# siboehm/ShallowSpeed

Hardware: AMD Instinct MI355X
Metric: samples/sec (whole node), 4-layer MLP MNIST-shape, DP×PP at 1/2/4/8 GPUs (higher is better)
Workload: dtype bf16; 1 GPU; model=mlp4_mnist_784x256x256x256x10, global_batch=16384, parallelism=dp1, schedule=naive, loss=xent, mubatches=1, hipgraph=False, fp8_fwd=False, deterministic=False

## Files before the change

csrc/bindings.cpp:

```cpp

#include <torch/extension.h>

#include <ATen/cuda/CUDAContext.h>

#include <climits>
#include <optional>
#include <string>

#include "launchers.h"

namespace {

hipStream_t cur_stream() {
    return (hipStream_t)at::cuda::getCurrentCUDAStream().stream();
}

void check_bf16(const torch::Tensor& t, const char* name) {
    TORCH_CHECK(t.is_cuda(), name, " must be on GPU");
    TORCH_CHECK(t.scalar_type() == torch::kBFloat16, name, " must be bf16");
    TORCH_CHECK(t.is_contiguous(), name, " must be contiguous");
}

void check_f32(const torch::Tensor& t, const char* name) {
    TORCH_CHECK(t.is_cuda(), name, " must be on GPU");
// ... 168 lines not shown
                                          const torch::Tensor& bsc,
                                          const torch::Tensor& bias,
                                          bool relu) {
    TORCH_CHECK(a.scalar_type() == torch::kUInt8 &&
                b.scalar_type() == torch::kUInt8, "a/b must be u8 (e4m3)");
    TORCH_CHECK(a.is_contiguous() && b.is_contiguous() &&
                asc.is_contiguous() && bsc.is_contiguous(), "contiguous");
    const int M = a.size(0), K = a.size(1), N = b.size(0);
    TORCH_CHECK(b.size(1) == K, "K mismatch");
    const void* bias_p = opt_bf16(bias, "bias");
    std::vector<torch::Tensor> out;
    bool ok;
    if (quantized) {
        out = {torch::empty({M, N}, a.options()),
               torch::empty({N / 128, M, 4}, a.options())};
        ok = ss_gemm_nt_f8_q(a.data_ptr(), asc.data_ptr(), b.data_ptr(),
                             bsc.data_ptr(), bias_p, out[0].data_ptr(),
                             out[1].data_ptr(), M, N, K, relu, cur_stream());
    } else {
        out = {torch::empty({M, N}, a.options().dtype(torch::kBFloat16))};
        ok = ss_gemm_nt_f8(a.data_ptr(), asc.data_ptr(), b.data_ptr(),
                           bsc.data_ptr(), bias_p, out[0].data_ptr(), M, N, K,
                           relu, cur_stream());
    }
    TORCH_CHECK(ok, "shape outside the fp8 tier: ", M, "x", N, "x", K);
    return out;
}

torch::Tensor gemm_nt_f8(torch::Tensor a, torch::Tensor asc, torch::Tensor b,
                         torch::Tensor bsc, torch::Tensor bias, bool relu) {
    return gemm_nt_f8_any(false, a, asc, b, bsc, bias, relu)[0];
}

std::vector<torch::Tensor> gemm_nt_f8_q(torch::Tensor a, torch::Tensor asc,
                                         torch::Tensor b, torch::Tensor bsc,
                                         torch::Tensor bias, bool relu) {
    return gemm_nt_f8_any(true, a, asc, b, bsc, bias, relu);
}

void wgrad_tn_256(torch::Tensor dy, torch::Tensor x, torch::Tensor gw) {
    check_bf16(dy, "dy");
    check_bf16(x, "x");
    check_f32(gw, "gw");
    const int Kb = dy.size(0), Mo = dy.size(1), N = x.size(1);
    TORCH_CHECK(x.size(0) == Kb, "batch mismatch");
    TORCH_CHECK(gw.size(0) == Mo && gw.size(1) == N, "gw shape");
    TORCH_CHECK(ss_wgrad_tn_256(dy.data_ptr(), x.data_ptr(), gw.data_ptr(),
                                Mo, N, Kb, cur_stream()),
                "shape outside the 256-tile wgrad tier");
}

void wgrad_tn(torch::Tensor dy, torch::Tensor x, torch::Tensor gw,
              torch::Tensor gb, torch::Tensor mask, int64_t split_k,
              int64_t stages) {
    check_bf16(dy, "dy");
    check_bf16(x, "x");
    check_f32(gw, "gw");
    const int Kb = dy.size(0), Mo = dy.size(1), N = x.size(1);
    TORCH_CHECK(x.size(0) == Kb, "batch mismatch");
    TORCH_CHECK(gw.size(0) == Mo && gw.size(1) == N, "gw shape");
    const void* mask_p = opt_bf16(mask, "mask");
    TORCH_CHECK(!mask_p || mask.sizes() == dy.sizes(), "mask must match dy");
    void* gb_p = opt_f32(gb, "gb");
    TORCH_CHECK(!gb_p || gb.numel() == Mo, "gb size");
    TORCH_CHECK(stages >= 0 && stages <= 2, "stages must be 0, 1 or 2");
    ss_wgrad_tn(dy.data_ptr(), x.data_ptr(), mask_p, gw.data_ptr(), gb_p, Mo,
                N, Kb, (int)split_k, (int)stages, cur_stream());
}

void wgrad_tn_multi(torch::Tensor chunk_table, int64_t nchunks,
                    bool has_mask, torch::Tensor gw, torch::Tensor gb,
                    int64_t Mo, int64_t N, int64_t kb_chunk,
                    int64_t split_k) {
    check_table(chunk_table, 3, "chunk_table must be CUDA int64 [nchunks,3]");
    TORCH_CHECK(chunk_table.size(0) == nchunks,
                "chunk_table must be CUDA int64 [nchunks,3]");
    check_f32(gw, "gw");
    TORCH_CHECK(gw.size(0) == Mo && gw.size(1) == N, "gw shape");
    void* gb_p = opt_f32(gb, "gb");
    TORCH_CHECK(!gb_p || gb.numel() == Mo, "gb size");
    ss_wgrad_tn_multi(chunk_table.data_ptr(), (int)nchunks, has_mask,
                      gw.data_ptr(), gb_p, (int)Mo, (int)N, (int)kb_chunk,
                      (int)split_k, cur_stream());
}

torch::Tensor colsum(torch::Tensor dy, torch::Tensor mask) {
    check_bf16(dy, "dy");
    const void* mask_p = opt_bf16(mask, "mask");
    auto gb = torch::zeros({dy.size(1)},
                           dy.options().dtype(torch::kFloat));
    ss_colsum(dy.data_ptr(), mask_p, gb.data_ptr(), dy.size(0), dy.size(1),
              cur_stream());
    return gb;
}

torch::Tensor relu_fwd(torch::Tensor x, std::optional<torch::Tensor> out) {
    check_bf16(x, "x");
    auto y = out_like(x, out);
    ss_relu_fwd(x.data_ptr(), y.data_ptr(), x.numel(), cur_stream());
    return y;
}

torch::Tensor relu_bwd(torch::Tensor dy, torch::Tensor y,
                       std::optional<torch::Tensor> out) {
    check_bf16(dy, "dy");
    check_bf16(y, "y");
    TORCH_CHECK(dy.sizes() == y.sizes(), "shape mismatch");
    auto dx = out_like(dy, out);
    ss_relu_bwd(dy.data_ptr(), y.data_ptr(), dx.data_ptr(), dy.numel(),
                cur_stream());
    return dx;
}

torch::Tensor relu_bwd_scaled(torch::Tensor dy, torch::Tensor y,
                              double scale,
                              std::optional<torch::Tensor> out) {
    check_bf16(dy, "dy");
    check_bf16(y, "y");
    TORCH_CHECK(dy.sizes() == y.sizes(), "shape mismatch");
    auto dx = out_like(dy, out);
    ss_relu_bwd_scaled(dy.data_ptr(), y.data_ptr(), dx.data_ptr(), dy.numel(),
                       (float)scale, cur_stream());
    return dx;
}

torch::Tensor softmax_fwd(torch::Tensor x) {
    check_bf16(x, "x");
    TORCH_CHECK(x.dim() == 2, "x must be 2-D");
    auto s = torch::empty_like(x);
    ss_softmax_fwd(x.data_ptr(), s.data_ptr(), x.size(0), x.size(1),
                   cur_stream());
    return s;
}

torch::Tensor softmax_bwd(torch::Tensor dy, torch::Tensor s) {
    check_bf16(dy, "dy");
    check_bf16(s, "s");
    TORCH_CHECK(dy.sizes() == s.sizes(), "shape mismatch");
    auto dx = torch::empty_like(dy);
    ss_softmax_bwd(dy.data_ptr(), s.data_ptr(), dx.data_ptr(), dy.size(0),
                   dy.size(1), cur_stream());
    return dx;
}

torch::Tensor head_mse_bwd(torch::Tensor s, torch::Tensor t,
                           double global_batch) {
    check_bf16(s, "probs");
    check_bf16(t, "target");
    TORCH_CHECK(s.sizes() == t.sizes(), "shape mismatch");
    auto dz = torch::empty_like(s);
    ss_head_mse_bwd(s.data_ptr(), t.data_ptr(), dz.data_ptr(), s.size(0),
                    s.size(1), (float)(1.0 / global_batch), cur_stream());
    return dz;
}

torch::Tensor head_xent_bwd(torch::Tensor s, torch::Tensor t,
                            double global_batch,
                            std::optional<torch::Tensor> out) {
    check_bf16(s, "probs");
    check_bf16(t, "target");
    TORCH_CHECK(s.sizes() == t.sizes(), "shape mismatch");
    auto dz = out_like(s, out);
    ss_head_xent_bwd(s.data_ptr(), t.data_ptr(), dz.data_ptr(), s.numel(),
                     (float)(1.0 / global_batch), cur_stream());
    return dz;
}
// ... 293 lines not shown

void adamw_multi(torch::Tensor desc, double lr, int64_t total, double beta1,
                 double beta2, double omb1, double omb2, double eps,
                 double weight_decay, double inv_bc1, double inv_bc2) {
    check_table(desc, 9, "desc must be CUDA int64 [T,9]");
    ss_adamw_multi(desc.data_ptr(), (int)desc.size(0), (long)total,
                   (float)lr, (float)beta1, (float)beta2, (float)omb1,
                   (float)omb2, (float)eps, (float)weight_decay,
                   (float)inv_bc1, (float)inv_bc2, cur_stream());
}

void sgd_multi2(torch::Tensor desc, torch::Tensor bmap, double lr,
                double momentum, double weight_decay) {
    check_table(desc, 8, "desc must be CUDA int64 [T,8]");
    check_table(bmap, 2, "bmap must be CUDA int64 [B,2]");
    ss_sgd_multi2(desc.data_ptr(), bmap.data_ptr(), (int)bmap.size(0),
                  (float)lr, (float)momentum, (float)weight_decay,
                  cur_stream());
}

void adamw_multi2(torch::Tensor desc, torch::Tensor bmap, double lr,
                  double beta1, double beta2, double omb1, double omb2,
                  double eps, double weight_decay, double inv_bc1,
                  double inv_bc2) {
    check_table(desc, 9, "desc must be CUDA int64 [T,9]");
    check_table(bmap, 2, "bmap must be CUDA int64 [B,2]");
    ss_adamw_multi2(desc.data_ptr(), bmap.data_ptr(), (int)bmap.size(0),
                    (float)lr, (float)beta1, (float)beta2, (float)omb1,
                    (float)omb2, (float)eps, (float)weight_decay,
                    (float)inv_bc1, (float)inv_bc2, cur_stream());
}

torch::Tensor fused_mlp_argmax(torch::Tensor x, torch::Tensor desc,
                               int64_t in_dim, int64_t nhidden,
                               int64_t cout) {
    check_bf16(x, "x");
    TORCH_CHECK(desc.is_cuda() && desc.scalar_type() == torch::kLong &&
                    desc.is_contiguous() &&
                    desc.numel() == (nhidden + 1) * 2,
                "desc must be CUDA int64 [(nhidden+1)*2]");
    const int M = x.size(0);
    TORCH_CHECK(x.size(1) == in_dim, "in_dim mismatch");
    auto out = torch::empty({M}, x.options().dtype(torch::kInt32));
    TORCH_CHECK(ss_fused_mlp_fwd(x.data_ptr(), desc.data_ptr(), M,
                                 (int)in_dim, (int)nhidden, (int)cout,
                                 out.data_ptr(), cur_stream()),
                "shape outside the fused-MLP tier");
    return out;
}

void transpose_bf16(torch::Tensor src, torch::Tensor dst) {
    check_bf16(src, "src");
    check_bf16(dst, "dst");
    const int rows = src.size(0), cols = src.size(1);
    TORCH_CHECK(src.dim() == 2 && dst.dim() == 2 &&
                    dst.size(0) == cols && dst.size(1) == rows &&
                    rows % 64 == 0 && cols % 64 == 0,
                "transpose_bf16 needs 64-aligned 2-D shapes");
    ss_transpose_bf16(src.data_ptr(), dst.data_ptr(), rows, cols,
                      cur_stream());
}

}

PYBIND11_MODULE(TORCH_EXTENSION_NAME, m) {
    m.def("gemm_nt", &gemm_nt, "C = A @ B^T (+bias)(+relu) with optional A-mask");
    m.def("gemm_nt_256", &gemm_nt_256,
          "256-tile 8-phase GEMM (M%256==N%256==K%128==0)");
    m.def("gemm_nt_256w", &gemm_nt_256w,
          "256-tile 8-phase GEMM, 4-wave 128x128-wave-tile variant");
    m.def("wgrad_tn_256", &wgrad_tn_256,
          "256-tile 8-phase wgrad: gw += dy^T @ x (no mask/bias)");
    m.def("fp8_quantize", &fp8_quantize,
          "bf16 [R,K] -> (e4m3 u8 [R,K], e8m0 scales [K/128,R,4])");
    m.def("gemm_nt_f8", &gemm_nt_f8,
          "MX-fp8 256-tile GEMM: C=bf16(A@B^T) (+bias)(+relu)");
    m.def("gemm_nt_f8_q", &gemm_nt_f8_q,
          "MX-fp8 GEMM with FUSED output quantization -> (e4m3, scales)");
    m.def("wgrad_tn", &wgrad_tn,
          "gW += (dy⊙mask)^T @ x; gb += colsum (fused); stages = LDS "
          "staging sets of the K loop (0 = the launcher's choice)",
          py::arg("dy"), py::arg("x"), py::arg("gw"), py::arg("gb"),
          py::arg("mask"), py::arg("split_k"), py::arg("stages") = 0);
    m.def("colsum", &colsum, "standalone column sum (bias grad)");
    m.def("wgrad_tn_multi", &wgrad_tn_multi,
          "chunked (deferred-µbatch) wgrad: one launch, many (dy,x) pairs");
    m.def("relu_fwd", &relu_fwd, py::arg("x"), py::arg("out") = py::none());
    m.def("relu_bwd", &relu_bwd, py::arg("dy"), py::arg("y"),
          py::arg("out") = py::none());
    m.def("relu_bwd_scaled", &relu_bwd_scaled,
          "dz = bf16(dy * scale) where y > 0, else +0", py::arg("dy"),
          py::arg("y"), py::arg("scale"), py::arg("out") = py::none());
    m.def("gemm_nt_dropout", &gemm_nt_dropout,
          "C = dropout(relu(A @ B^T + bias)), mask in the GEMM epilogue",
          py::arg("a"), py::arg("b"), py::arg("bias"), py::arg("key0"),
          py::arg("key1"), py::arg("step"), py::arg("layer"),
          py::arg("row_first"), py::arg("row_stride"), py::arg("thr"),
          py::arg("scale"), py::arg("fused") = true);
    m.def("dropout_fwd_", &dropout_fwd_,
          "in-place dropout of a finished post-ReLU activation");
    m.def("dropout_keep_mask", &dropout_keep_mask,
          "keep bits (bool [M][ncols]) for explicit sample ids");
    m.def("softmax_fwd", &softmax_fwd);
    m.def("softmax_bwd", &softmax_bwd);
    m.def("head_mse_bwd", &head_mse_bwd);
    m.def("head_xent_bwd", &head_xent_bwd, py::arg("probs"),
          py::arg("target"), py::arg("global_batch"),
          py::arg("out") = py::none());
    m.def("head_fwd_fused", &head_fwd_fused,
          "fused head forward: softmax(bf16(x @ w^T + b))", py::arg("x"),
          py::arg("w"), py::arg("b"), py::arg("rows_per_block") = 0);
    m.def("head_bwd_fused", &head_bwd_fused,
          "fused head backward -> (dz, dx); optional gW/gb accumulate",
          py::arg("probs"), py::arg("target"), py::arg("x"), py::arg("w_t"),
          py::arg("global_batch"), py::arg("grad_w"), py::arg("grad_b"),
          py::arg("rows_per_block") = 0,
          py::arg("metrics") = py::none(), py::arg("slots") = 0);
    m.def("bwd_chain", &bwd_chain,
          "head backward + 256-wide ReLU dgrads in one launch -> "
          "[dz_head, dz_l..., (dx)], or [] outside the contract",
          py::arg("probs"), py::arg("target"), py::arg("w_head_t"),
          py::arg("global_batch"), py::arg("hs"), py::arg("w_ts"),
          py::arg("rows") = 0, py::arg("waves") = 0, py::arg("w_lds") = 0,
          py::arg("dz_scale") = 1.0);
    m.def("fwd_chain", &fwd_chain,
          "256-wide ReLU layers + fused head forward in one launch -> "
          "[h_l..., probs], or [] outside the contract",
          py::arg("x"), py::arg("ws"), py::arg("bs"), py::arg("w_head"),
          py::arg("b_head"), py::arg("rows") = 0, py::arg("waves") = 0,
          py::arg("l1") = 0, py::arg("kloop") = 0,
          py::arg("zero") = py::none());
    m.def("head_metrics", &head_metrics,
          "metric totals of (probs, target) into a slotted accumulator",
          py::arg("probs"), py::arg("target"), py::arg("acc"),
          py::arg("kind") = "xent");
    m.def("sgd_multi", &sgd_multi);
    m.def("adamw_multi", &adamw_multi);
    m.def("transpose_bf16", &transpose_bf16);
    m.def("sgd_multi2", &sgd_multi2);
    m.def("adamw_multi2", &adamw_multi2);
    m.def("fused_mlp_argmax", &fused_mlp_argmax,
          "persistent fused MLP forward + per-row argmax (serving)");
    m.def("ln_fwd", &ln_fwd);
    m.def("ln_bwd_dx", &ln_bwd_dx);
    m.def("ln_bwd_dparam", &ln_bwd_dparam);
    m.def("gelu_fwd", &gelu_fwd, py::arg("z"), py::arg("out") = py::none());
    m.def("gelu_bwd", &gelu_bwd, py::arg("dy"), py::arg("z"),
          py::arg("out") = py::none());
    m.def("row_argmax", &row_argmax);
}
```

csrc/launchers.h:

```cpp
#pragma once

#include <hip/hip_runtime.h>

#include <cstdint>

inline bool aligned16(const void* p) { return p && ((uintptr_t)p & 15) == 0; }

void ss_gemm_nt(const void* A, const void* B, const void* bias,
                const void* mask, void* C, int M, int N, int K, bool relu,
                hipStream_t stream);
void ss_colsum(const void* dY, const void* mask, void* gb, int M, int N,
               hipStream_t stream);

struct DropoutArgs {
    unsigned key0, key1;
    unsigned layer, step;
    unsigned row_first, row_stride;
    unsigned thr;
    float scale;
};
bool ss_gemm_nt_dropout(const void* A, const void* B, const void* bias,
                        void* C, int M, int N, int K,
                        const DropoutArgs& drop, hipStream_t stream);

bool ss_gemm_nt_256(const void* A, const void* B, const void* bias, void* C,
                    int M, int N, int K, bool relu, hipStream_t stream);
bool ss_gemm_nt_256w(const void* A, const void* B, const void* bias, void* C,
                     int M, int N, int K, bool relu, hipStream_t stream);

void ss_fp8_quantize(const void* X, void* Q, void* S, int R, int K,
                     hipStream_t stream);
bool ss_gemm_nt_f8(const void* A, const void* Asc, const void* B,
                   const void* Bsc, const void* bias, void* C, int M, int N,
                   int K, bool relu, hipStream_t stream);
bool ss_gemm_nt_f8_q(const void* A, const void* Asc, const void* B,
                     const void* Bsc, const void* bias, void* Cq, void* Cs,
                     int M, int N, int K, bool relu, hipStream_t stream);

void ss_wgrad_tn(const void* dY, const void* X, const void* mask, void* gW,
                 void* gb, int Mo, int N, int Kb, int split_k, int stages,
                 hipStream_t stream);
void ss_wgrad_tn_multi(const void* chunk_table, int nchunks, bool has_mask,
                       void* gW, void* gb, int Mo, int N, int Kb_chunk,
                       int split_k, hipStream_t stream);
bool ss_wgrad_tn_256(const void* dY, const void* X, void* gW, int Mo, int N,
                     int Kb, hipStream_t stream);

bool ss_head_fwd_fused(const void* x, const void* W, const void* bias,
                       void* probs, int M, int K, int C, int rows_per_block,
                       hipStream_t stream);
bool ss_head_bwd_fused(const void* probs, const void* target, const void* x,
                       const void* Wt, void* dz, void* dx, void* gW, void* gb,
                       int M, int K, int C, float inv_gb, int rows_per_block,
                       void* metrics, int slots, hipStream_t stream);
bool ss_head_metrics(const void* probs, const void* target, void* acc,
                     int slots, int M, int C, int kind, hipStream_t stream);

constexpr int SS_BWD_CHAIN_MAX = 8;
bool ss_bwd_chain(const void* probs, const void* target, const void* Wt_head,
                  void* dz_head, const void* const* h, const void* const* wt,
                  void* const* dz, int nlayers, void* dx, int M, int H, int C,
                  float inv_gb, int rows, int waves, int w_lds,
                  float dz_scale, hipStream_t stream);

constexpr int SS_FWD_CHAIN_MAX = 8;
bool ss_fwd_chain(const void* x, const void* const* w, const void* const* b,
                  void* const* h, int nlayers, const void* W_head,
                  const void* b_head, void* probs, int M, int K0, int H, int C,
                  int rows, int waves, int l1, int kloop, void* zero_ptr,
                  long zero_bytes, hipStream_t stream);

bool ss_fused_mlp_fwd(const void* x, const void* desc, int M, int in_dim,
                      int nhidden, int cout, void* out, hipStream_t stream);

void ss_relu_fwd(const void* x, void* y, long n, hipStream_t stream);
void ss_relu_bwd(const void* dy, const void* y, void* dx, long n,
                 hipStream_t stream);
void ss_relu_bwd_scaled(const void* dy, const void* y, void* dx, long n,
                        float scale, hipStream_t stream);
void ss_dropout_fwd(void* y, int M, int N, const DropoutArgs& drop,
                    hipStream_t stream);
void ss_dropout_mask(const void* sample_ids, void* keep, int M, int N,
                     const DropoutArgs& drop, hipStream_t stream);
void ss_softmax_fwd(const void* x, void* s, int B, int C, hipStream_t stream);
void ss_softmax_bwd(const void* dy, const void* s, void* dx, int B, int C,
                    hipStream_t stream);
void ss_head_mse_bwd(const void* s, const void* t, void* dz, int B, int C,
                     float inv_gb, hipStream_t stream);
void ss_head_xent_bwd(const void* s, const void* t, void* dz, long n,
                      float inv_gb, hipStream_t stream);
void ss_row_argmax(const void* x, void* out, int B, int C,
                   hipStream_t stream);
void ss_transpose_bf16(const void* src, void* dst, int rows, int cols,
                       hipStream_t stream);
void ss_sgd_multi(const void* desc, int ntensors, long total, float lr,
                  float momentum, float weight_decay, hipStream_t stream);
void ss_adamw_multi(const void* desc, int ntensors, long total, float lr,
                    float beta1, float beta2, float omb1, float omb2,
                    float eps, float weight_decay, float inv_bc1,
                    float inv_bc2, hipStream_t stream);
void ss_sgd_multi2(const void* desc, const void* bmap, int nblocks, float lr,
                   float momentum, float weight_decay, hipStream_t stream);
void ss_adamw_multi2(const void* desc, const void* bmap, int nblocks,
                     float lr, float beta1, float beta2, float omb1,
                     float omb2, float eps, float weight_decay,
                     float inv_bc1, float inv_bc2, hipStream_t stream);

void ss_ln_fwd(const void* x, const void* gamma, const void* beta, void* y,
               void* mean, void* rstd, int B, int C, float eps,
               hipStream_t stream);
void ss_ln_bwd_dx(const void* dy, const void* x, const void* gamma,
                  const void* mean, const void* rstd, void* dx, int B, int C,
                  hipStream_t stream);
void ss_ln_bwd_dparam(const void* dy, const void* x, const void* mean,
                      const void* rstd, void* dgamma, void* dbeta, int B,
                      int C, hipStream_t stream);
void ss_gelu_fwd(const void* z, void* y, long n, hipStream_t stream);
void ss_gelu_bwd(const void* dy, const void* z, void* dz, long n,
                 hipStream_t stream);
```

csrc/wgrad.hip:

```cpp

#include "common.h"
#include "launchers.h"
#include "wgrad_dev.h"

#define WGRAD_DECODE                                                        \
    const int gx = gridDim.x, gy = gridDim.y;                               \
    const int nwg = gx * gy * gridDim.z;                                    \
    const int hw = blockIdx.x + gx * (blockIdx.y + gy * blockIdx.z);        \
    const int wid = xcd_remap(hw, nwg);                                     \
    const int bidy = wid % gy;                                              \
    const int bidx = (wid / gy) % gx;                                       \
    int bidz = wid / (gy * gx);                                             \
    if (chunks) {                                                           \
        const long* row = chunks + (long)(bidz / nsplit) * 3;               \
        dY = (const __bf16*)row[0];                                         \
        X = (const __bf16*)row[1];                                          \
        mask = (const __bf16*)row[2];                                       \
        bidz = bidz % nsplit;                                               \
    }                                                                       \
    const gbf16* const gdY = (const gbf16*)dY;                              \
    const gbf16* const gX = (const gbf16*)X;                                \
    const gbf16* const gmask = (const gbf16*)mask;                          \
    const int m0 = bidx * BMT;                                              \
    const int n0 = bidy * BNT;                                              \
    const int kbeg = bidz * k_per_split;                                    \
    const int kend = min(Kb, kbeg + k_per_split);
#define WGRAD_DB_OWNER bidy == 0

template <int BMT, int BNT, bool HAS_MASK, int KG, int NSTAGE>
__global__ __launch_bounds__(KG * 256, BMT* BNT > 64 * 64 ? 2 : 4)
void wgrad_tn_kernel(
    const __bf16* __restrict__ dY,
    const __bf16* __restrict__ X,
    const __bf16* __restrict__ mask,
    float* __restrict__ gW,
    float* __restrict__ gb,
    int Mo, int N, int Kb, int k_per_split,
    const long* __restrict__ chunks, int nsplit) {
    __shared__ __attribute__((aligned(16)))
    ushort smem[NSTAGE * wgrad_set_el<BMT, BNT, KG>()];
#define WGRAD_TILE_HERE
#include "wgrad_dev.h"
}
#undef WGRAD_DECODE
#undef WGRAD_DB_OWNER


namespace {

constexpr int WGRAD_KG_128 = 2;
constexpr int WGRAD_KG_64 = 4;
constexpr int WGRAD_TARGET_BLOCKS = 256;

struct WgradCfg {
    int bm, bn, kg;
};

WgradCfg wgrad_cfg(int Mo, int N, int split_k) {
    int tile = ((Mo >= 256 && N >= 512) || (Mo >= 512 && N >= 256)) ? 1 : 0;
    static const int env_big = env_int("SS_WGRAD_BIG", -1);
    static const int env_kg = env_int("SS_WGRAD_KG", -1);
    if (env_big >= 0) tile = env_big > 2 ? 1 : env_big;
    WgradCfg c;
    c.bm = tile == 1 ? 128 : 64;
    c.bn = tile == 0 ? 64 : 128;
    c.kg = tile == 0 ? WGRAD_KG_64 : WGRAD_KG_128;
    if (env_kg == 1 || env_kg == 2 || env_kg == 4) c.kg = env_kg;
    if (tile != 0 && c.kg > 2) c.kg = 2;
    if (split_k == 1) c.kg = 1;
    return c;
}

int wgrad_auto_split(int tiles, int Kb, int kg) {
    static const int env_blocks = env_int("SS_WGRAD_BLOCKS", 0);
    const int target = env_blocks > 0 ? env_blocks : WGRAD_TARGET_BLOCKS;
    int split_k = cdiv(target, tiles);
    while (split_k & (split_k - 1)) split_k &= split_k - 1;
    const int max_split = cdiv(Kb, 64 * kg);
    if (split_k > max_split) split_k = max_split;
    return split_k;
}

int wgrad_stages(const WgradCfg& cfg, int Mo, int N, bool has_mask,
                 int stages) {
    if (stages == 1 || stages == 2) return stages;
    static const int env_stages = env_int("SS_WGRAD_STAGES", 0);
    if (env_stages == 1 || env_stages == 2) return env_stages;
    return !has_mask && cfg.kg > 1 && Mo >= cfg.bm && N >= cfg.bn ? 2 : 1;
}

}

#define WGRAD_LAUNCH(BMT, BNT, HM, KGV, ...)                                \
    do {                                                                    \
        if (stages == 2)                                                    \
            hipLaunchKernelGGL((wgrad_tn_kernel<BMT, BNT, HM, KGV, 2>),     \
                               grid, dim3(KGV * 256), 0, stream,            \
                               __VA_ARGS__);                                \
        else                                                                \
            hipLaunchKernelGGL((wgrad_tn_kernel<BMT, BNT, HM, KGV, 1>),     \
                               grid, dim3(KGV * 256), 0, stream,            \
                               __VA_ARGS__);                                \
    } while (0)
#define WGRAD_BY_MASK(BMT, BNT, KGV, ...)                                   \
    do {                                                                    \
        if (has_mask) WGRAD_LAUNCH(BMT, BNT, true, KGV, __VA_ARGS__);       \
        else WGRAD_LAUNCH(BMT, BNT, false, KGV, __VA_ARGS__);               \
    } while (0)
#define WGRAD_DISPATCH(cfg, ...)                                            \
    do {                                                                    \
        if (cfg.bm == 128) {                                                \
            if (cfg.kg == 1) WGRAD_BY_MASK(128, 128, 1, __VA_ARGS__);       \
            else WGRAD_BY_MASK(128, 128, 2, __VA_ARGS__);                   \
        } else if (cfg.bn == 128) {                                         \
            if (cfg.kg == 1) WGRAD_BY_MASK(64, 128, 1, __VA_ARGS__);        \
            else WGRAD_BY_MASK(64, 128, 2, __VA_ARGS__);                    \
        } else {                                                            \
            if (cfg.kg == 1) WGRAD_BY_MASK(64, 64, 1, __VA_ARGS__);         \
            else if (cfg.kg == 2) WGRAD_BY_MASK(64, 64, 2, __VA_ARGS__);    \
            else WGRAD_BY_MASK(64, 64, 4, __VA_ARGS__);                     \
        }                                                                   \
    } while (0)

void ss_wgrad_tn(const void* dY, const void* X, const void* mask, void* gW,
                 void* gb, int Mo, int N, int Kb, int split_k, int stages,
                 hipStream_t stream) {
    if (!mask && split_k <= 0 && Mo >= 512 && N >= 512 &&
        (long)(Mo / 256) * (N / 256) >= 64) {
        static const int en = env_int("SS_WGRAD256", 1);
        if (en && ss_wgrad_tn_256(dY, X, gW, Mo, N, Kb, stream)) {
            if (gb) ss_colsum(dY, nullptr, gb, Kb, Mo, stream);
            return;
        }
    }
    const WgradCfg cfg = wgrad_cfg(Mo, N, split_k);
    if (split_k <= 0)
        split_k = wgrad_auto_split(cdiv(Mo, cfg.bm) * cdiv(N, cfg.bn), Kb,
                                   cfg.kg);
    int k_per_split = cdiv(cdiv(Kb, split_k), 64) * 64;
    split_k = cdiv(Kb, k_per_split);
    dim3 grid(cdiv(Mo, cfg.bm), cdiv(N, cfg.bn), split_k);
    const bool has_mask = mask != nullptr;
    stages = wgrad_stages(cfg, Mo, N, has_mask, stages);
    WGRAD_DISPATCH(cfg, (const __bf16*)dY, (const __bf16*)X,
                   (const __bf16*)mask, (float*)gW, (float*)gb, Mo, N, Kb,
                   k_per_split, (const long*)nullptr, 1);
}

void ss_wgrad_tn_multi(const void* chunk_table, int nchunks, bool has_mask,
                       void* gW, void* gb, int Mo, int N, int Kb_chunk,
                       int split_k, hipStream_t stream) {
    const WgradCfg cfg = wgrad_cfg(Mo, N, split_k);
    if (split_k <= 0)
        split_k = wgrad_auto_split(
            cdiv(Mo, cfg.bm) * cdiv(N, cfg.bn) * nchunks, Kb_chunk, cfg.kg);
    int k_per_split = cdiv(cdiv(Kb_chunk, split_k), 64) * 64;
    split_k = cdiv(Kb_chunk, k_per_split);
    dim3 grid(cdiv(Mo, cfg.bm), cdiv(N, cfg.bn), split_k * nchunks);
    const int stages = 1;
    WGRAD_DISPATCH(cfg, (const __bf16*)nullptr, (const __bf16*)nullptr,
                   (const __bf16*)nullptr, (float*)gW, (float*)gb, Mo, N,
                   Kb_chunk, k_per_split, (const long*)chunk_table, split_k);
}
```

shallowspeed_amd/models/layers.py:

```python

import math

import torch

from ..ops import functional as F


_DZ_FIRST = None


def _dz_first_enabled() -> bool:
    global _DZ_FIRST
    if _DZ_FIRST is None:
        import os

        _DZ_FIRST = os.environ.get("SS_DZ_FIRST", "0") == "1"
    return _DZ_FIRST


def _shape_seed(in_dims: int, out_dims: int) -> int:
    return (in_dims * 1_000_003 + out_dims * 7919) & 0x7FFFFFFF


class Parameter:
# ... 501 lines not shown
        for hook in self._grad_hooks:
            for p in layer.parameters():
                if p.requires_grad:
                    hook(p)

    def _backward_head_fused(self, lin, head, target, mubatch_id):
        s = head._unstash("s", mubatch_id)
        x = lin._unstash("x", mubatch_id)
        if target.dtype != s.dtype:
            target = target.to(s.dtype)
        if not target.is_contiguous():
            target = target.contiguous()
        in_kernel = (F.head_wgrad_fused() and not lin._defer_wgrad
                     and not F.deterministic())
        acc = head._metrics if head._training else None
        if acc is not None and not F.head_metrics_fused():
            F.head_metrics(s, target, acc, head.kind)
            acc = None
        dz, dx = F.head_bwd_fused(
            s, target, x, lin.weight.compute_t(), head.global_batch_size,
            lin.weight.grad if in_kernel else None,
            lin.bias.grad if in_kernel else None, metrics=acc)
        if lin._defer_wgrad:
            lin._wgrad_pending.append((dz, x, None))
            if len(lin._wgrad_pending) >= lin._wgrad_window:
                lin.flush_wgrad()
        elif not in_kernel:
            F.linear_wgrad_acc(dz, x, lin.weight.grad, lin.bias.grad)
        self._fire_grad_hooks(head)
        self._fire_grad_hooks(lin)
        return dx

    def _bwd_chain_plan(self, mubatch_rows: int = 1):
        if mubatch_rows < 1 or not F.bwd_chain_enabled() \
                or not F.head_fused() or F.head_wgrad_fused() \
                or self._chain_head_pair() is None:
            return None
        plan = []
        for i in self._chain_run():
            layer = self.layers[i]
            need_dx = not (i == 0 and self._skip_input_grad)
            in_chain = need_dx and layer.in_dims == self._CHAIN_WIDTH
            if not in_chain and plan and not F.bwd_chain_dz_last():
                break
            plan.append((i, in_chain))
            if not in_chain:
                break
        if self._has_dropout and \
                len({self.layers[i].dz_scale() for i, _ in plan}) > 1:
            return None
        return plan or None

    def _wgrad_of(self, layer, dz, x):
        if layer._defer_wgrad:
            layer._wgrad_pending.append((dz, x, None))
            if len(layer._wgrad_pending) >= layer._wgrad_window:
                layer.flush_wgrad()
        else:
            F.linear_wgrad_acc(dz, x, layer.weight.grad, layer.bias.grad)

    def _backward_chain(self, plan, lin, head, target, mubatch_id):
        s = head._cache.get(("s", mubatch_id))
        x = lin._cache.get(("x", mubatch_id))
        chain = [self.layers[i] for i, _ in plan]
        hs = [l._cache.get(("y", mubatch_id)) for l in chain]
        if s is None or x is None or any(h is None for h in hs) \
                or not F.head_fused_ok(x, lin):
            return False, None
        if target.dtype != s.dtype:
            target = target.to(s.dtype)
        if not target.is_contiguous():
            target = target.contiguous()
        w_ts = [l.weight.compute_t() for l, (_, dg) in zip(chain, plan) if dg]
        res = F.bwd_chain(s, target, lin.weight.compute_t(),
                          head.global_batch_size, hs, w_ts,
                          dz_scale=chain[0].dz_scale())
        if res is None:
            return False, None
        dz_head, dzs, dx = res
        if head._metrics is not None and head._training:
            F.head_metrics(s, target, head._metrics, head.kind)
        head._unstash("s", mubatch_id)
        lin._unstash("x", mubatch_id)
        self._wgrad_of(lin, dz_head, x)
        self._fire_grad_hooks(head)
        self._fire_grad_hooks(lin)
        for layer, (i, dg), dz in zip(chain, plan, dzs):
            xl = layer._unstash("x", mubatch_id)
            layer._unstash("y", mubatch_id)
            if not dg and not (i == 0 and self._skip_input_grad):
                dx = F.linear_dgrad(dz, layer.weight.compute(),
                                    layer.weight.compute_t())
            self._wgrad_of(layer, dz, xl)
            self._fire_grad_hooks(layer)
        return True, dx

    def backward(self, dout, mubatch_id: int = 0):
        self._settle_zero_grad()
        d = dout
        last = len(self.layers) - 1
        pair = self._head_pair()
        plan = self._bwd_chain_plan(dout.shape[0]) \
            if pair and dout.is_cuda else None
        if plan:
            ok, dx = self._backward_chain(plan, pair[0], pair[1], d,
                                          mubatch_id)
            if ok:
                d = dx
                last = plan[-1][0] - 1
                pair = None
        if pair:
            lin, head = pair
            x = lin._cache.get(("x", mubatch_id))
            need_dx = not (last == 1 and self._skip_input_grad)
            if x is not None and need_dx and F.head_fused_ok(x, lin):
                d = self._backward_head_fused(lin, head, d, mubatch_id)
                last -= 2
        for i in range(last, -1, -1):
            layer = self.layers[i]
            if i == 0 and self._skip_input_grad and isinstance(layer, Linear):
                d = layer.backward(d, mubatch_id, need_dx=False)
            else:
                d = layer.backward(d, mubatch_id)
            self._fire_grad_hooks(layer)
        for hook in self._post_grad_hooks:
            hook(self.parameters())
        return d

    def register_grad_hook(self, fn):
        self._grad_hooks.append(fn)

    def reset_grad_hooks(self):
        self._grad_hooks = []

    def register_post_grad_hook(self, fn):
        self._post_grad_hooks.append(fn)

    def reset_post_grad_hooks(self):
        self._post_grad_hooks = []

    def parameters(self):
        return [p for layer in self.layers for p in layer.parameters()]

    def zero_grad(self, defer=False):
        flat = getattr(self, "_flat_grad", None)
        self._zero_pending = False
        if flat is None:
            for layer in self.layers:
                layer.zero_grad()
        elif defer and flat.is_cuda and F.fwd_zero_grads() \
                and self._fwd_chain_plan():
            self._zero_pending = True
        else:
            flat.zero_()

    def _settle_zero_grad(self):
        if getattr(self, "_zero_pending", False):
            self._zero_pending = False
            self._flat_grad.zero_()

    def train(self):
        self._training = True
        for l in self.layers:
            l.train()

    def eval(self):
        self._training = False
        for l in self.layers:
            l.eval()

    def set_metrics(self, acc):
        head = self.layers[-1] if self.layers else None
        if not isinstance(head, _LossHead):
            return False
        head._metrics = acc
        return True

    def set_fp8_fwd(self, flag: bool):
# ... 83 lines not shown
```

shallowspeed_amd/ops/functional.py:

```python

import functools

import torch

from ._ext import load_ext


_DETERMINISTIC = False


def set_deterministic(flag: bool):
    global _DETERMINISTIC
    _DETERMINISTIC = bool(flag)


def deterministic() -> bool:
    return _DETERMINISTIC


_HEAD_FUSED = None


def set_head_fused(flag: bool):
    global _HEAD_FUSED
# ... 96 lines not shown
    return _FWD_ZERO_GRADS


def _is_gpu(t: torch.Tensor) -> bool:
    return t.is_cuda


def _ext_for(t: torch.Tensor):
    return load_ext(required=True) if _is_gpu(t) else None



def linear_fwd(x, w, b=None, relu=False):
    if _is_gpu(x):
        ext = _ext_for(x)
        empty = torch.Tensor()
        return ext.gemm_nt(x, w, b if b is not None else empty, empty, bool(relu))
    y = x @ w.t()
    if b is not None:
        y = y + b
    if relu:
        y = torch.clamp(y, min=0)
    return y


def fp8_quantize(x):
    return _ext_for(x).fp8_quantize(x)


def linear_fwd_fp8(xq, xs, wq, ws, b=None, relu=False):
    ext = _ext_for(xq)
    empty = torch.Tensor()
    return ext.gemm_nt_f8(xq, xs, wq, ws, b if b is not None else empty,
                          bool(relu))


def linear_dgrad(dy, w, w_t=None, mask_src=None):
    if _is_gpu(dy):
        ext = _ext_for(dy)
        assert w_t is not None, "GPU dgrad needs the transposed weight copy"
        M, O = dy.shape
        if (mask_src is None and not _DETERMINISTIC
                and M >= 2048 and O >= 1024 and w.shape[1] >= 1024
                and _dgrad_lib_enabled()):
            return torch.matmul(dy, w_t.t())
        empty = torch.Tensor()
        return ext.gemm_nt(dy, w_t, empty, mask_src if mask_src is not None else empty, False)
    if mask_src is not None:
        dy = dy * (mask_src > 0).to(dy.dtype)
    return dy @ w


_DGRAD_LIB = None


def _dgrad_lib_enabled() -> bool:
    global _DGRAD_LIB
    if _DGRAD_LIB is None:
        import os

        _DGRAD_LIB = os.environ.get("SS_DGRAD_LIB", "1") == "1"
    return _DGRAD_LIB


def linear_wgrad_acc(dy, x, grad_w, grad_b=None, mask_src=None, split_k=0):
    if split_k == 0 and _DETERMINISTIC:
        split_k = 1
    if _is_gpu(dy):
        ext = _ext_for(dy)
        ext.wgrad_tn(
            dy,
            x,
            grad_w,
            grad_b if grad_b is not None else torch.Tensor(),
            mask_src if mask_src is not None else torch.Tensor(),
            int(split_k),
        )
        return
    if mask_src is not None:
        dy = dy * (mask_src > 0).to(dy.dtype)
    grad_w += (dy.t() @ x).to(grad_w.dtype)
    if grad_b is not None:
        grad_b += dy.sum(dim=0).to(grad_b.dtype)



def relu_fwd(x):
    if _is_gpu(x):
        return _ext_for(x).relu_fwd(x)
    return torch.where(x <= 0, torch.zeros_like(x), x)


def relu_bwd(dy, y, scale=1.0):
    if float(scale) == 1.0:
        if _is_gpu(dy):
            return _ext_for(dy).relu_bwd(dy, y)
        return torch.where(y > 0, dy, torch.zeros_like(dy))
    if _is_gpu(dy):
        return _ext_for(dy).relu_bwd_scaled(dy, y, float(scale))
    return torch.where(y > 0, dy * float(scale), torch.zeros_like(dy))



_PHILOX_M0, _PHILOX_M1 = 0xD2511F53, 0xCD9E8D57
_PHILOX_W0, _PHILOX_W1 = 0x9E3779B9, 0xBB67AE85
_U32 = 0xFFFFFFFF


def philox4x32_10(counter, key):
    import numpy as np

    c0, c1, c2, c3 = np.broadcast_arrays(
        *[np.asarray(c, dtype=np.uint64) for c in counter])
    k0, k1 = int(key[0]) & _U32, int(key[1]) & _U32
    m32 = np.uint64(_U32)
    s32 = np.uint64(32)
    for _ in range(10):
        p0 = np.uint64(_PHILOX_M0) * c0
        p1 = np.uint64(_PHILOX_M1) * c2
        c0, c1, c2, c3 = ((p1 >> s32) ^ c1 ^ np.uint64(k0), p1 & m32,
                          (p0 >> s32) ^ c3 ^ np.uint64(k1), p0 & m32)
        k0 = (k0 + _PHILOX_W0) & _U32
        k1 = (k1 + _PHILOX_W1) & _U32
    return c0, c1, c2, c3


@functools.lru_cache(maxsize=64)
def dropout_params(p):
    import numpy as np

    p = float(p)
    if not 0.0 <= p < 1.0:
        raise ValueError(f"dropout p must be in [0, 1), got {p}")
    thr = min(_U32, int(np.floor((1.0 - p) * 4294967296.0 + 0.5)))
    return thr, float(np.float32(1.0 / (1.0 - p)))


def _seed_words(seed):
    seed = int(seed)
    assert 0 <= seed < 1 << 64, "dropout seed is 64 bits"
    return seed & _U32, seed >> 32


def dropout_keep_mask(seed, step, layer, sample_ids, ncols, p):
    import numpy as np

    thr, _ = dropout_params(p)
    k0, k1 = _seed_words(seed)
    step, layer, ncols = int(step), int(layer), int(ncols)
    assert 0 <= step <= _U32 and 0 <= layer <= _U32 and ncols >= 0
    if not torch.is_tensor(sample_ids):
        sample_ids = torch.as_tensor(list(sample_ids), dtype=torch.int64)
    sample_ids = sample_ids.to(torch.int64).reshape(-1)
    if sample_ids.numel():
        assert int(sample_ids.min()) >= 0 and \
            int(sample_ids.max()) <= _U32, "sample id must be < 2^32"
    if _is_gpu(sample_ids):
        return _ext_for(sample_ids).dropout_keep_mask(
            sample_ids.contiguous(), ncols, k0, k1, step, layer, thr)
    ngroups = (ncols + 3) // 4
    s = sample_ids.numpy().astype(np.uint64)[:, None]
    g = np.arange(ngroups, dtype=np.uint64)[None, :]
    words = philox4x32_10((s, g, np.uint64(layer), np.uint64(step)),
                          (k0, k1))
    w = np.stack(words, axis=-1).reshape(s.shape[0], ngroups * 4)[:, :ncols]
    return torch.from_numpy(w < np.uint64(thr))
# ... 297 lines not shown
```

Baseline: 138.2 million samples/sec.

## Group per-layer weight-gradient GEMMs of the backward chain into shared launches

Adds a grouped wgrad kernel that takes up to eight (dy, x, gW, gb) problems sharing one tile configuration and launches them as a single grid. Each block decodes its problem from a table of block offsets, and a planner rebalances split-K across problems toward a target block count. The fused backward chain now collects the head and hidden-layer wgrads and issues them through this path by default, which removes per-launch overhead and fills the GPU better for small 256-wide layers. The cost is grad hooks firing later, a branchy per-block decode, and split choices that may differ from the single-problem heuristic.

```diff
diff --git a/csrc/bindings.cpp b/csrc/bindings.cpp
--- a/csrc/bindings.cpp
+++ b/csrc/bindings.cpp
@@ -274,6 +274,79 @@
     ss_wgrad_tn_multi(chunk_table.data_ptr(), (int)nchunks, has_mask,
                       gw.data_ptr(), gb_p, (int)Mo, (int)N, (int)kb_chunk,
                       (int)split_k, cur_stream());
+}
+
+using WgradGroupProblem = std::tuple<torch::Tensor, torch::Tensor,
+                                     torch::Tensor,
+                                     std::optional<torch::Tensor>>;
+
+std::vector<int> wgrad_group_splits(
+    const std::optional<std::vector<int64_t>>& splits, size_t n) {
+    std::vector<int> s(n, 0);
+    if (!splits) return s;
+    TORCH_CHECK(splits->size() == n, "splits: one per problem");
+    for (size_t i = 0; i < n; ++i) {
+        const int64_t v = (*splits)[i];
+        TORCH_CHECK(v == 0 || (v >= 2 && v <= INT_MAX),
+                    "split must be 0 (the group rule) or >= 2");
+        s[i] = (int)v;
+    }
+    return s;
+}
+
+void wgrad_tn_group(std::vector<WgradGroupProblem> problems,
+                    std::optional<std::vector<int64_t>> splits) {
+    std::vector<WgradProblem> p;
+    for (const auto& [dy, x, gw, gb] : problems) {
+        check_bf16(dy, "dy");
+        check_bf16(x, "x");
+        check_f32(gw, "gw");
+        TORCH_CHECK(dy.dim() == 2 && x.dim() == 2 && gw.dim() == 2,
+                    "dy, x, gw must be 2-D");
+        const int Kb = dy.size(0), Mo = dy.size(1), N = x.size(1);
+        TORCH_CHECK(x.size(0) == Kb, "batch mismatch");
+        TORCH_CHECK(gw.size(0) == Mo && gw.size(1) == N, "gw shape");
+        void* gb_p = gb ? opt_f32(*gb, "gb") : nullptr;
+        TORCH_CHECK(!gb_p || gb->numel() == Mo, "gb size");
+        p.push_back({dy.data_ptr(), x.data_ptr(), gw.data_ptr(), gb_p, Mo, N,
+                     Kb});
+    }
+    const std::vector<int> s = wgrad_group_splits(splits, p.size());
+    if (p.empty()) return;
+    TORCH_CHECK(ss_wgrad_tn_group(p.data(), (int)p.size(), s.data(),
+                                  cur_stream()),
+                "wgrad_tn_group: bad shape, split or pointer");
+}
+
+std::vector<std::tuple<std::vector<int64_t>, std::vector<int64_t>,
+                       std::vector<int64_t>>>
+wgrad_group_plan(std::vector<std::tuple<int64_t, int64_t, int64_t>> shapes,
+                 std::optional<std::vector<int64_t>> splits) {
+    std::vector<WgradProblem> p;
+    for (const auto& [Kb, Mo, N] : shapes) {
+        TORCH_CHECK(Kb >= 1 && Mo >= 1 && N >= 1 && Kb <= INT_MAX &&
+                        Mo <= INT_MAX && N <= INT_MAX,
+                    "shape (Kb, Mo, N)");
+        p.push_back({nullptr, nullptr, nullptr, nullptr, (int)Mo, (int)N,
+                     (int)Kb});
+    }
+    const std::vector<int> s = wgrad_group_splits(splits, p.size());
+    std::vector<WgradGroupLaunch> plan(p.size());
+    const int nl =
+        ss_wgrad_group_plan(p.data(), (int)p.size(), s.data(), plan.data());
+    TORCH_CHECK(nl >= 0, "wgrad_group_plan: bad shape or split");
+    std::vector<std::tuple<std::vector<int64_t>, std::vector<int64_t>,
+                           std::vector<int64_t>>> out;
+    for (int l = 0; l < nl; ++l) {
+        std::vector<int64_t> idx, sp, bl;
+        for (int k = 0; k < plan[l].count; ++k) {
+            idx.push_back(plan[l].first + k);
+            sp.push_back(plan[l].split[k]);
+            bl.push_back(plan[l].blocks[k]);
+        }
+        out.emplace_back(idx, sp, bl);
+    }
+    return out;
 }
 
 torch::Tensor colsum(torch::Tensor dy, torch::Tensor mask) {
@@ -733,6 +806,14 @@
           "staging sets of the K loop (0 = the launcher's choice)",
           py::arg("dy"), py::arg("x"), py::arg("gw"), py::arg("gb"),
           py::arg("mask"), py::arg("split_k"), py::arg("stages") = 0);
+    m.def("wgrad_tn_group", &wgrad_tn_group,
+          "unmasked wgrads of a list of (dy, x, gw, gb): consecutive "
+          "problems of one tile configuration share a launch",
+          py::arg("problems"), py::arg("splits") = py::none());
+    m.def("wgrad_group_plan", &wgrad_group_plan,
+          "launches of wgrad_tn_group for (Kb, Mo, N) shapes: per launch "
+          "(problem indices, splits, block counts)",
+          py::arg("shapes"), py::arg("splits") = py::none());
     m.def("colsum", &colsum, "standalone column sum (bias grad)");
     m.def("wgrad_tn_multi", &wgrad_tn_multi,
           "chunked (deferred-µbatch) wgrad: one launch, many (dy,x) pairs");
diff --git a/csrc/launchers.h b/csrc/launchers.h
--- a/csrc/launchers.h
+++ b/csrc/launchers.h
@@ -45,6 +45,24 @@
                        int split_k, hipStream_t stream);
 bool ss_wgrad_tn_256(const void* dY, const void* X, void* gW, int Mo, int N,
                      int Kb, hipStream_t stream);
+
+constexpr int SS_WGRAD_GROUP_MAX = 8;
+struct WgradProblem {
+    const void* dY;
+    const void* X;
+    void* gW;
+    void* gb;
+    int Mo, N, Kb;
+};
+struct WgradGroupLaunch {
+    int first, count;
+    int split[SS_WGRAD_GROUP_MAX];
+    int blocks[SS_WGRAD_GROUP_MAX];
+};
+int ss_wgrad_group_plan(const WgradProblem* problems, int n,
+                        const int* splits, WgradGroupLaunch* out);
+bool ss_wgrad_tn_group(const WgradProblem* problems, int n,
+                       const int* splits, hipStream_t stream);
 
 bool ss_head_fwd_fused(const void* x, const void* W, const void* bias,
                        void* probs, int M, int K, int C, int rows_per_block,
diff --git a/csrc/wgrad.hip b/csrc/wgrad.hip
--- a/csrc/wgrad.hip
+++ b/csrc/wgrad.hip
@@ -2,6 +2,9 @@
 #include "common.h"
 #include "launchers.h"
 #include "wgrad_dev.h"
+
+#include <climits>
+#include <vector>
 
 #define WGRAD_DECODE                                                        \
     const int gx = gridDim.x, gy = gridDim.y;                               \
@@ -45,6 +48,69 @@
 #undef WGRAD_DECODE
 #undef WGRAD_DB_OWNER
 
+struct WgradGroupItem {
+    const __bf16* dY;
+    const __bf16* X;
+    float* gW;
+    float* gb;
+    int Mo, N, Kb, k_per_split;
+    int gx, gy;
+    int first;
+};
+struct WgradGroupArgs {
+    WgradGroupItem p[SS_WGRAD_GROUP_MAX];
+};
+
+using gf32 = __attribute__((address_space(1))) float;
+
+#define WGRAD_DECODE                                                        \
+    const int wid = xcd_remap((int)blockIdx.x, (int)gridDim.x);             \
+    const gbf16* gdY = (const gbf16*)args.p[0].dY;                          \
+    const gbf16* gX = (const gbf16*)args.p[0].X;                            \
+    gf32* sgW = (gf32*)args.p[0].gW;                                        \
+    gf32* sgb = (gf32*)args.p[0].gb;                                        \
+    int Mo = args.p[0].Mo, N = args.p[0].N, Kb = args.p[0].Kb;              \
+    int k_per_split = args.p[0].k_per_split;                                \
+    int gx = args.p[0].gx, gy = args.p[0].gy, first = 0;                    \
+    _Pragma("unroll") for (int i = 1; i < SS_WGRAD_GROUP_MAX; ++i) {        \
+        const bool t = wid >= args.p[i].first;                              \
+        gdY = t ? (const gbf16*)args.p[i].dY : gdY;                         \
+        gX = t ? (const gbf16*)args.p[i].X : gX;                            \
+        sgW = t ? (gf32*)args.p[i].gW : sgW;                                \
+        sgb = t ? (gf32*)args.p[i].gb : sgb;                                \
+        Mo = t ? args.p[i].Mo : Mo;                                         \
+        N = t ? args.p[i].N : N;                                            \
+        Kb = t ? args.p[i].Kb : Kb;                                         \
+        k_per_split = t ? args.p[i].k_per_split : k_per_split;              \
+        gx = t ? args.p[i].gx : gx;                                         \
+        gy = t ? args.p[i].gy : gy;                                         \
+        first = t ? args.p[i].first : first;                                \
+    }                                                                       \
+    float* const gW = (float*)sgW;                                          \
+    float* const gb = (float*)sgb;                                          \
+    const gbf16* const gmask = nullptr;                                     \
+    const int lid = wid - first;                                            \
+    const int bidy = lid % gy;                                              \
+    const int bidx = (lid / gy) % gx;                                       \
+    const int bidz = lid / (gy * gx);                                       \
+    const int m0 = bidx * BMT;                                              \
+    const int n0 = bidy * BNT;                                              \
+    const int kbeg = bidz * k_per_split;                                    \
+    const int kend = min(Kb, kbeg + k_per_split);
+#define WGRAD_DB_OWNER bidy == 0
+
+template <int BMT, int BNT, int KG, int NSTAGE>
+__global__ __launch_bounds__(KG * 256, BMT* BNT > 64 * 64 ? 2 : 4)
+void wgrad_group_kernel(const WgradGroupArgs args) {
+    constexpr bool HAS_MASK = false;
+    __shared__ __attribute__((aligned(16)))
+    ushort smem[NSTAGE * wgrad_set_el<BMT, BNT, KG>()];
+#define WGRAD_TILE_HERE
+#include "wgrad_dev.h"
+}
+#undef WGRAD_DECODE
+#undef WGRAD_DB_OWNER
+
 
 namespace {
 
@@ -71,9 +137,13 @@
     return c;
 }
 
+int wgrad_target_blocks() {
+    static const int env_blocks = env_int("SS_WGRAD_BLOCKS", 0);
+    return env_blocks > 0 ? env_blocks : WGRAD_TARGET_BLOCKS;
+}
+
 int wgrad_auto_split(int tiles, int Kb, int kg) {
-    static const int env_blocks = env_int("SS_WGRAD_BLOCKS", 0);
-    const int target = env_blocks > 0 ? env_blocks : WGRAD_TARGET_BLOCKS;
+    const int target = wgrad_target_blocks();
     int split_k = cdiv(target, tiles);
     while (split_k & (split_k - 1)) split_k &= split_k - 1;
     const int max_split = cdiv(Kb, 64 * kg);
@@ -87,6 +157,56 @@
     static const int env_stages = env_int("SS_WGRAD_STAGES", 0);
     if (env_stages == 1 || env_stages == 2) return env_stages;
     return !has_mask && cfg.kg > 1 && Mo >= cfg.bm && N >= cfg.bn ? 2 : 1;
+}
+
+bool wgrad_tier256(int Mo, int N, int split_k) {
+    static const int en = env_int("SS_WGRAD256", 1);
+    return en && split_k <= 0 && Mo >= 512 && N >= 512 &&
+           (long)(Mo / 256) * (N / 256) >= 64;
+}
+
+bool wgrad_groupable(const WgradCfg& c) {
+    return (c.bm == 64 && c.bn == 64 && c.kg == 4) ||
+           (c.bn == 128 && c.kg == 2);
+}
+
+int wgrad_eff_split(int Kb, int split_k) {
+    return cdiv(Kb, cdiv(cdiv(Kb, split_k), 64) * 64);
+}
+
+void wgrad_group_splits(int n, const int* tiles, const int* Kb, int kg,
+                        int* split) {
+    const int target = wgrad_target_blocks();
+    bool autos[SS_WGRAD_GROUP_MAX];
+    int blocks = 0;
+    for (int i = 0; i < n; ++i) {
+        autos[i] = split[i] == 0;
+        if (autos[i]) split[i] = wgrad_auto_split(tiles[i] * n, Kb[i], kg);
+        split[i] = wgrad_eff_split(Kb[i], split[i]);
+        blocks += tiles[i] * split[i];
+    }
+    if (n < 2) return;
+    for (;;) {
+        int best = -1, best_s = 0;
+        for (int i = 0; i < n; ++i) {
+            if (!autos[i]) continue;
+            const int max_split = cdiv(Kb[i], 64 * kg);
+            int s = split[i] + 1;
+            while (s <= max_split && wgrad_eff_split(Kb[i], s) == split[i])
+                ++s;
+            if (s > max_split) continue;
+            s = wgrad_eff_split(Kb[i], s);
+            if (blocks + tiles[i] * (s - split[i]) > target) continue;
+            if (best < 0 || cdiv(Kb[i], split[i]) >
+                                cdiv(Kb[best], split[best])) {
+                best = i;
+                best_s = s;
+            }
+        }
+        if (best < 0) return;
+        blocks += tiles[best] * (best_s - split[best]);
+        split[best] = best_s;
+    }
 }
 
 }
@@ -125,10 +245,8 @@
 void ss_wgrad_tn(const void* dY, const void* X, const void* mask, void* gW,
                  void* gb, int Mo, int N, int Kb, int split_k, int stages,
                  hipStream_t stream) {
-    if (!mask && split_k <= 0 && Mo >= 512 && N >= 512 &&
-        (long)(Mo / 256) * (N / 256) >= 64) {
-        static const int en = env_int("SS_WGRAD256", 1);
-        if (en && ss_wgrad_tn_256(dY, X, gW, Mo, N, Kb, stream)) {
+    if (!mask && wgrad_tier256(Mo, N, split_k)) {
+        if (ss_wgrad_tn_256(dY, X, gW, Mo, N, Kb, stream)) {
             if (gb) ss_colsum(dY, nullptr, gb, Kb, Mo, stream);
             return;
         }
@@ -162,3 +280,107 @@
                    (const __bf16*)nullptr, (float*)gW, (float*)gb, Mo, N,
                    Kb_chunk, k_per_split, (const long*)chunk_table, split_k);
 }
+
+
+int ss_wgrad_group_plan(const WgradProblem* p, int n, const int* splits,
+                        WgradGroupLaunch* out) {
+    if (n < 0 || (n > 0 && (!p || !out))) return -1;
+    for (int i = 0; i < n; ++i) {
+        if (p[i].Mo < 1 || p[i].N < 1 || p[i].Kb < 1) return -1;
+        if (splits && (splits[i] < 0 || splits[i] == 1)) return -1;
+    }
+    auto split_of = [&](int i) { return splits ? splits[i] : 0; };
+    auto cfg_of = [&](int i) {
+        return wgrad_cfg(p[i].Mo, p[i].N, split_of(i));
+    };
+    auto can_group = [&](int i) {
+        return wgrad_groupable(cfg_of(i)) &&
+               !wgrad_tier256(p[i].Mo, p[i].N, split_of(i));
+    };
+    int nl = 0;
+    for (int i = 0; i < n;) {
+        const WgradCfg cfg = cfg_of(i);
+        int j = i + 1;
+        if (can_group(i)) {
+            for (; j < n && j - i < SS_WGRAD_GROUP_MAX && can_group(j); ++j) {
+                const WgradCfg c = cfg_of(j);
+                if (c.bm != cfg.bm || c.bn != cfg.bn || c.kg != cfg.kg) break;
+            }
+        }
+        WgradGroupLaunch& L = out[nl++];
+        L = WgradGroupLaunch{};
+        L.first = i;
+        L.count = j - i;
+        auto tiles_of = [&](int k) {
+            return cdiv(p[k].Mo, cfg.bm) * cdiv(p[k].N, cfg.bn);
+        };
+        if (L.count == 1 && wgrad_tier256(p[i].Mo, p[i].N, split_of(i))) {
+            i = j;
+            continue;
+        }
+        int tiles[SS_WGRAD_GROUP_MAX], kb[SS_WGRAD_GROUP_MAX];
+        for (int k = i; k < j; ++k) {
+            tiles[k - i] = tiles_of(k);
+            kb[k - i] = p[k].Kb;
+            L.split[k - i] = split_of(k);
+        }
+        wgrad_group_splits(L.count, tiles, kb, cfg.kg, L.split);
+        for (int k = i; k < j; ++k)
+            L.blocks[k - i] = tiles[k - i] * L.split[k - i];
+        i = j;
+    }
+    return nl;
+}
+
+bool ss_wgrad_tn_group(const WgradProblem* p, int n, const int* splits,
+                       hipStream_t stream) {
+    if (n == 0) return true;
+    std::vector<WgradGroupLaunch> plan(n > 0 ? n : 0);
+    const int nl = ss_wgrad_group_plan(p, n, splits, plan.data());
+    if (nl < 0) return false;
+    for (int i = 0; i < n; ++i)
+        if (!aligned16(p[i].dY) || !aligned16(p[i].X) || !p[i].gW ||
+            ((uintptr_t)p[i].gW & 3) || ((uintptr_t)p[i].gb & 3))
+            return false;
+    for (int l = 0; l < nl; ++l) {
+        const WgradGroupLaunch& L = plan[l];
+        const WgradProblem* q = p + L.first;
+        if (L.count == 1) {
+            ss_wgrad_tn(q->dY, q->X, nullptr, q->gW, q->gb, q->Mo, q->N,
+                        q->Kb, splits ? splits[L.first] : 0, 0, stream);
+            continue;
+        }
+        const WgradCfg cfg = wgrad_cfg(q->Mo, q->N, 0);
+        WgradGroupArgs args;
+        int nblocks = 0;
+        for (int k = 0; k < SS_WGRAD_GROUP_MAX; ++k) {
+            WgradGroupItem& it = args.p[k];
+            it = WgradGroupItem{};
+            it.first = INT_MAX;
+            if (k >= L.count) continue;
+            it.dY = (const __bf16*)q[k].dY;
+            it.X = (const __bf16*)q[k].X;
+            it.gW = (float*)q[k].gW;
+            it.gb = (float*)q[k].gb;
+            it.Mo = q[k].Mo;
+            it.N = q[k].N;
+            it.Kb = q[k].Kb;
+            it.k_per_split = cdiv(cdiv(q[k].Kb, L.split[k]), 64) * 64;
+            it.gx = cdiv(q[k].Mo, cfg.bm);
+            it.gy = cdiv(q[k].N, cfg.bn);
+            it.first = nblocks;
+            nblocks += L.blocks[k];
+        }
+        const dim3 grid(nblocks);
+        if (cfg.bm == 128)
+            hipLaunchKernelGGL((wgrad_group_kernel<128, 128, 2, 2>), grid,
+                               dim3(2 * 256), 0, stream, args);
+        else if (cfg.bn == 128)
+            hipLaunchKernelGGL((wgrad_group_kernel<64, 128, 2, 2>), grid,
+                               dim3(2 * 256), 0, stream, args);
+        else
+            hipLaunchKernelGGL((wgrad_group_kernel<64, 64, 4, 2>), grid,
+                               dim3(4 * 256), 0, stream, args);
+    }
+    return true;
+}
diff --git a/shallowspeed_amd/models/layers.py b/shallowspeed_amd/models/layers.py
--- a/shallowspeed_amd/models/layers.py
+++ b/shallowspeed_amd/models/layers.py
@@ -607,18 +607,43 @@
             F.head_metrics(s, target, head._metrics, head.kind)
         head._unstash("s", mubatch_id)
         lin._unstash("x", mubatch_id)
-        self._wgrad_of(lin, dz_head, x)
-        self._fire_grad_hooks(head)
-        self._fire_grad_hooks(lin)
+        grouped = F.wgrad_group_enabled() and not F.deterministic() \
+            and not any(l._defer_wgrad for l in [lin] + chain)
+        items = [(lin, dz_head, x, (head, lin))]
+        if not grouped:
+            self._wgrad_of(lin, dz_head, x)
+            self._fire_grad_hooks(head)
+            self._fire_grad_hooks(lin)
         for layer, (i, dg), dz in zip(chain, plan, dzs):
             xl = layer._unstash("x", mubatch_id)
             layer._unstash("y", mubatch_id)
             if not dg and not (i == 0 and self._skip_input_grad):
                 dx = F.linear_dgrad(dz, layer.weight.compute(),
                                     layer.weight.compute_t())
+            if grouped:
+                items.append((layer, dz, xl, (layer,)))
+                continue
             self._wgrad_of(layer, dz, xl)
             self._fire_grad_hooks(layer)
+        if grouped:
+            self._wgrad_group(items)
         return True, dx
+
+    def _wgrad_group(self, items):
+        probs = [(dz, x, l.weight.grad, l.bias.grad) for l, dz, x, _ in items]
+        if not self._grad_hooks:
+            cuts = [list(range(len(items)))]
+        elif probs[0][0].is_cuda:
+            cuts = [la["problems"] for la in F.wgrad_group_plan(
+                [(dz.shape[0], dz.shape[1], x.shape[1])
+                 for dz, x, _, _ in probs])]
+        else:
+            cuts = [[k] for k in range(len(items))]
+        for cut in cuts:
+            F.linear_wgrad_group([probs[k] for k in cut])
+            for k in cut:
+                for hl in items[k][3]:
+                    self._fire_grad_hooks(hl)
 
     def backward(self, dout, mubatch_id: int = 0):
         self._settle_zero_grad()
diff --git a/shallowspeed_amd/ops/functional.py b/shallowspeed_amd/ops/functional.py
--- a/shallowspeed_amd/ops/functional.py
+++ b/shallowspeed_amd/ops/functional.py
@@ -202,6 +202,44 @@
     grad_w += (dy.t() @ x).to(grad_w.dtype)
     if grad_b is not None:
         grad_b += dy.sum(dim=0).to(grad_b.dtype)
+
+
+_WGRAD_GROUP = None
+
+
+def set_wgrad_group(flag: bool):
+    global _WGRAD_GROUP
+    _WGRAD_GROUP = bool(flag)
+
+
+def wgrad_group_enabled() -> bool:
+    global _WGRAD_GROUP
+    if _WGRAD_GROUP is None:
+        import os
+
+        _WGRAD_GROUP = os.environ.get("SS_WGRAD_GROUP", "1") != "0"
+    return _WGRAD_GROUP
+
+
+def wgrad_group_plan(shapes, splits=None):
+    ext = load_ext(required=True)
+    return [dict(problems=list(i), splits=list(s), blocks=list(b))
+            for i, s, b in ext.wgrad_group_plan(
+                [tuple(int(v) for v in sh) for sh in shapes],
+                None if splits is None else [int(s) for s in splits])]
+
+
+def linear_wgrad_group(problems, splits=None):
+    problems = list(problems)
+    if not problems:
+        return
+    if _is_gpu(problems[0][0]):
+        load_ext(required=True).wgrad_tn_group(
+            [tuple(p) for p in problems],
+            None if splits is None else [int(s) for s in splits])
+        return
+    for dy, x, gw, gb in problems:
+        linear_wgrad_acc(dy, x, gw, gb)
 
 
 
```

After: 152.3 million samples/sec (median of 6 runs). +10.1%, better.
